# SparseBLAS/spblas-reference

Measured on AMD Instinct MI355X. Metric: csr_spmv_gflops, higher is better.
Workload: dtype f32; 1 GPU; cfg2: fp32 CSR SpMV 10000000x10000000, exactly 10 nnz/row, uniform random unsorted columns, int32 indices, nnz=100000000; rows=10000000, cols=10000000, nnz=100000000, index_type=int32, parallelism=single GPU, operand=matrix_opt(csr_view) + multiply_inspect, alg=auto, plan_alg=3, plan_bytes=1204259164

## Files before the change

spblas-reference_amd/csrc/spmv_sliced.hip:

```cpp
#include <algorithm>
#include <atomic>
#include <type_traits>
#include <vector>

#include "common.hpp"
#include "plan.hpp"
#include "scan.hpp"

#include <cstdlib>
#include <ctime>

namespace spb {

int spmv_hot_build(spblas_gfx950_handle_t h, spblas_gfx950_plan_s* pl, const void* values, bool auto_mode);
int spmv_hot_exec(spblas_gfx950_handle_t h, spblas_gfx950_plan_s* pl, const void* alpha, const void* x, const void* beta,
                  void* y);
int spmv_hot_rows(spblas_gfx950_handle_t h, spblas_gfx950_plan_s* pl, const void* alpha, const void* x, void* y);
int spmv_hot_update(spblas_gfx950_handle_t h, spblas_gfx950_plan_s* pl, const void* values);
void spmv_hot_free(spblas_gfx950_handle_t h, spblas_gfx950_plan_s* pl);
void spmv_sliced_free(spblas_gfx950_handle_t h, spblas_gfx950_plan_s* pl);

static int env_int(const char* name, int dflt) {
  const char* v = std::getenv(name);
  return v && *v ? std::atoi(v) : dflt;
// ... 1468 lines not shown
      }
    }
  };
  if (g_hi > g_lo) {
    batch_t qa, qb;
    issue(g_lo, qa);
    for (int g = g_lo; g < g_hi; g += 2 * UB) {
      issue(g + UB, qb);
      consume(g, qa);
      issue(g + 2 * UB, qa);
      consume(g + UB, qb);
    }
  }
  if (dbg & 2)
    *dummy = dbg_sum;
  if (ENC8 && item.y == 0 && !(dbg & 3)) {
    const int ne = exc_cnt[wb];
    for (int i = lane; i < ne; i += 64) {
      const unsigned e = exc_idx[(size_t) wb * exc_cap + i];
      unsafeAtomicAdd(acc + exc_row[(size_t) wb * exc_cap + i], P[e]);
    }
  }
  if (partial) {
    T* dst = ritems ? partial : partial + (int64_t) blockIdx.y * pstride + r0;
    for (int i0 = lane; i0 < rh; i0 += 64 * 8) {
      T v[8];
#pragma unroll
      for (int u = 0; u < 8; ++u)
        v[u] = acc[i0 + 64 * u < rh ? i0 + 64 * u : 0];
#pragma unroll
      for (int u = 0; u < 8; ++u)
        if (i0 + 64 * u < rh)
          dst[i0 + 64 * u] = v[u];
    }
    return;
  }
  if (peers) {
    for (int i0 = lane; i0 < rh; i0 += 64 * 8) {
      T v[8];
#pragma unroll
      for (int u = 0; u < 8; ++u)
        v[u] = alpha * acc[i0 + 64 * u < rh ? i0 + 64 * u : 0];
      for (int p = 0; p < n_peers; ++p) {
        T* dst = peers[p] + peer_off + r0;
#pragma unroll
        for (int u = 0; u < 8; ++u)
          if (i0 + 64 * u < rh)
            dst[i0 + 64 * u] = v[u];
      }
    }
    return;
  }
  if (rowmap) {
    for (int i = lane; i < rh; i += 64) {
      const T v = alpha * acc[i];
      const int32_t r = rowmap[r0 + i];
      if (r < 0)
        piece_out[r0 + i] = v;
      else
        y[r] = beta == T(0) ? v : v + beta * y[r];
    }
    return;
  }
  for (int i0 = lane; i0 < rh; i0 += 64 * 8) {
    T v[8];
#pragma unroll
    for (int u = 0; u < 8; ++u) {
      const int i = i0 + 64 * u;
      v[u] = alpha * acc[i < rh ? i : 0];
    }
#pragma unroll
    for (int u = 0; u < 8; ++u) {
      const int i = i0 + 64 * u;
      if (i < rh)
        y[r0 + i] = beta == T(0) ? v[u] : v[u] + beta * y[r0 + i];
    }
  }
}


#ifndef PB_VF_GLDS_AUX
#define PB_VF_GLDS_AUX 2
#endif
template <typename T, int NW, int UB, bool ENC8>
__global__ __launch_bounds__(NW * 64) void pb_reduce_vf_kernel(int64_t m, int Hw, int64_t wb_begin, int64_t wb_end,
                                                               const int32_t* __restrict__ binblk, const T* __restrict__ P,
                                                               const uint16_t* __restrict__ s_row,
                                                               const uint16_t* __restrict__ s_src,
                                                               const T* __restrict__ values, const void* __restrict__ rowptr,
                                                               int o64, T* __restrict__ y, T alpha, T beta, int win_cap,
                                                               const typename pb_hdr<T>::type* __restrict__ s_hdr,
                                                               const unsigned* __restrict__ exc_idx,
                                                               const uint16_t* __restrict__ exc_row,
                                                               const int32_t* __restrict__ exc_cnt, int exc_cap,
                                                               T* const* __restrict__ peers, int n_peers, int64_t peer_off) {
  extern __shared__ __attribute__((aligned(16))) unsigned char smem[];
  const int tid = threadIdx.x, wave = __builtin_amdgcn_readfirstlane(threadIdx.x >> 6), lane = threadIdx.x & 63;
  T* win = reinterpret_cast<T*>(smem);
  T* const acc0 = win + win_cap;
  T* const acc = acc0 + (size_t) wave * (Hw + 64);
  const int64_t stride = gridDim.x;
  int64_t wb = wb_begin + blockIdx.x;
  if (wb >= wb_end)
    return;
  constexpr int PB_GBLK = pb_geom<T>::GBLK;
  constexpr int LPB = pb_geom<T>::BLK / 4;
  constexpr int VE = 16 / (int) sizeof(T);
  typedef typename pb_hdr<T>::type hdr_t;
  struct batch_t {
    T p[UB][4];
    u16x4 s[UB];
    u16x4 r[UB];
    unsigned cw[UB];
    hdr_t hd[UB];
  };
  T* const dummy = acc + Hw + lane;
  auto row_off = [&](int64_t r) -> int64_t {
    return o64 ? (int64_t) static_cast<const int64_t*>(rowptr)[r] : (int64_t) static_cast<const int32_t*>(rowptr)[r];
  };
  auto wave_range = [&](int64_t b, int& lo, int& hi) {
    const int gb0 = binblk[b] / PB_GBLK, ng = binblk[b + 1] / PB_GBLK - gb0;
    lo = gb0 + (int) ((int64_t) ng * wave / NW);
    hi = gb0 + (int) ((int64_t) ng * (wave + 1) / NW);
  };
  auto issue = [&](int g, int last, batch_t& q) {
#pragma unroll
    for (int u = 0; u < UB; ++u) {
      const int gg = (g + u) < last ? (g + u) : last;
      const unsigned offR = ((unsigned) gg * PB_GRP + 4u * (unsigned) lane) * 2u;
      const unsigned offP = offR * (unsigned) (sizeof(T) / 2);
      pack4<T>::load(reinterpret_cast<const T*>(reinterpret_cast<const char*>(P) + offP), q.p[u]);
      q.s[u] = stream_load(reinterpret_cast<const u16x4*>(reinterpret_cast<const char*>(s_src) + offR));
      if (ENC8) {
        q.cw[u] = stream_load(reinterpret_cast<const unsigned*>(reinterpret_cast<const char*>(s_row) + (offR >> 1)));
        q.hd[u] = stream_load(s_hdr + ((unsigned) gg * (unsigned) PB_GBLK + (unsigned) lane / LPB));
      } else {
        q.r[u] = stream_load(reinterpret_cast<const u16x4*>(reinterpret_cast<const char*>(s_row) + offR));
      }
    }
  };
  int shift = 0;
  auto stage_window = [&](int64_t b) {
#ifdef PB_EXP_VF_NOWIN
    return;
#endif
    const int64_t r0 = b * Hw, r1 = (r0 + Hw) < m ? (r0 + Hw) : m;
    const int64_t p0 = row_off(r0), p1 = row_off(r1);
    const bool vec_ok = (reinterpret_cast<uintptr_t>(values) & 15) == 0;
    const int64_t p_lo = vec_ok ? (p0 & ~(int64_t) (VE - 1)) : p0;
    shift = (int) (p0 - p_lo);
    const int wn = (int) (p1 - p_lo);
    if (vec_ok) {
      typedef T vec_t __attribute__((ext_vector_type(VE)));
      const int nv = wn / VE;
      const vec_t* src = reinterpret_cast<const vec_t*>(values + p_lo);
      const int nchunk = (nv + 63) >> 6;
      for (int c = wave; c < nchunk; c += NW) {
        const int i = c * 64 + lane;
        if (i < nv)
          __builtin_amdgcn_global_load_lds((const __attribute__((address_space(1))) void*) (src + i),
                                           (__attribute__((address_space(3))) void*) (reinterpret_cast<vec_t*>(win) + c * 64),
                                           16, 0, PB_VF_GLDS_AUX);
      }
      for (int i = nv * VE + tid; i < wn; i += NW * 64)
        win[i] = stream_load(values + p_lo + i);
    } else {
      for (int i = tid; i < wn; i += NW * 64)
        win[i] = stream_load(values + p_lo + i);
    }
  };
  auto consume = [&](int g, int g_hi, const batch_t& q) {
    const T* wv = win + shift;
#pragma unroll
    for (int u = 0; u < UB; ++u) {
      if (g + u >= g_hi)
        break;
#ifdef PB_EXP_VF_NOACC
      {
        T t = q.p[u][0] + q.p[u][1] + q.p[u][2] + q.p[u][3] + T(q.s[u][0] ^ q.s[u][1] ^ q.s[u][2] ^ q.s[u][3]);
        if (ENC8)
          t += T(q.cw[u] ^ (unsigned) q.hd[u]);
        else
          t += T(q.r[u][0]);
        *dummy += t;
        continue;
      }
#endif
      T v[4], pr[4];
      T* slot[4];
      bool flagged[4], atomic[4];
#pragma unroll
      for (int j = 0; j < 4; ++j)
        pr[j] = wv[q.s[u][j]];
      if (ENC8) {
        unsigned row[4];
        bool skip[4];
        pb_decode_rows<LPB>(q.cw[u], pb_hdr<T>::base(q.hd[u]), lane, (unsigned) Hw, row, skip);
        const unsigned fl = pb_hdr<T>::flags(q.hd[u]) >> (4 * (lane & (LPB - 1)));
#pragma unroll
        for (int j = 0; j < 4; ++j) {
          atomic[j] = ((fl >> j) & 1u) != 0 && !skip[j];
          flagged[j] = atomic[j] || skip[j];
          slot[j] = acc + row[j];
          v[j] = *slot[j];
        }
      } else {
#pragma unroll
        for (int j = 0; j < 4; ++j) {
          unsigned r = q.r[u][j];
          asm("" : "+v"(r));
          flagged[j] = atomic[j] = r > 0x7FFFu;
          slot[j] = acc + (r & 0x7FFFu);
          v[j] = *slot[j];
        }
      }
#pragma unroll
      for (int j = 0; j < 4; ++j) {
        pr[j] *= q.p[u][j];
        T* w = flagged[j] ? dummy : slot[j];
        *w = v[j] + pr[j];
      }
      if (__builtin_amdgcn_ballot_w64(atomic[0] | atomic[1] | atomic[2] | atomic[3]) != 0) {
#pragma unroll
        for (int j = 0; j < 4; ++j)
          if (atomic[j])
            unsafeAtomicAdd(slot[j], pr[j]);
      }
    }
  };
  auto end_of_bin = [&]() {
    if (ENC8 && wave == 0) {
      const T* wv = win + shift;
      const int ne = exc_cnt[wb];
      for (int i = lane; i < ne; i += 64) {
        const unsigned e = exc_idx[(size_t) wb * exc_cap + i];
        unsafeAtomicAdd(acc + exc_row[(size_t) wb * exc_cap + i], P[e] * wv[s_src[e]]);
      }
    }
    __builtin_amdgcn_s_waitcnt(0xc07f);
    __builtin_amdgcn_s_barrier();
    const int64_t r0 = wb * Hw;
    const int rh = (int) (((r0 + Hw) < m ? (r0 + Hw) : m) - r0);
    for (int i0 = tid; i0 < rh; i0 += NW * 64 * 4) {
      T sum[4];
#pragma unroll
      for (int u = 0; u < 4; ++u) {
        const int i = (i0 + u * NW * 64) < rh ? (i0 + u * NW * 64) : 0;
        T t = acc0[i];
#pragma unroll
        for (int w = 1; w < NW; ++w)
          t += acc0[(size_t) w * (Hw + 64) + i];
        sum[u] = alpha * t;
      }
#pragma unroll
      for (int u = 0; u < 4; ++u) {
        const int i = i0 + u * NW * 64;
        if (i < rh) {
          if (peers) {
            for (int p = 0; p < n_peers; ++p)
              peers[p][peer_off + r0 + i] = sum[u];
          } else {
            y[r0 + i] = beta == T(0) ? sum[u] : sum[u] + beta * y[r0 + i];
          }
#pragma unroll
          for (int w = 0; w < NW; ++w)
            acc0[(size_t) w * (Hw + 64) + i] = T(0);
        }
      }
    }
    wb += stride;
    if (wb < wb_end) {
      stage_window(wb);
      __builtin_amdgcn_s_waitcnt(0);
      __builtin_amdgcn_s_barrier();
    }
  };
  batch_t qa, qb;
  int g_lo, g_hi;
  wave_range(wb, g_lo, g_hi);
  issue(g_lo, g_hi > g_lo ? g_hi - 1 : g_lo, qa);
  for (int i = tid; i < NW * (Hw + 64); i += NW * 64)
    acc0[i] = T(0);
  stage_window(wb);
  __builtin_amdgcn_s_waitcnt(0);
  __builtin_amdgcn_s_barrier();
  for (;;) {
    const int64_t nb = wb + stride;
    int n_lo = g_hi > g_lo ? g_hi - 1 : g_lo, n_hi = n_lo;
    if (nb < wb_end)
      wave_range(nb, n_lo, n_hi);
    const int last = g_hi > g_lo ? g_hi - 1 : g_lo, n_last = n_hi > n_lo ? n_hi - 1 : n_lo;
    int g = g_lo;
    do {
      issue(g + UB, last, qb);
      consume(g, g_hi, qa);
      const bool more = g + 2 * UB < g_hi;
      issue(more ? g + 2 * UB : n_lo, more ? last : n_last, qa);
      consume(g + UB, g_hi, qb);
      g += 2 * UB;
    } while (g < g_hi);
    end_of_bin();
    if (wb >= wb_end)
      break;
    g_lo = n_lo;
    g_hi = n_hi;
  }
}

template <typename T>
static const void* pb_reduce_vf_fn(int nw, int ub, bool enc8) {
#define SPB_VF(NW_, UB_, E_) reinterpret_cast<const void*>(pb_reduce_vf_kernel<T, NW_, UB_, E_>)
  if (enc8) {
    if (nw == 8)
      return ub == 4 ? SPB_VF(8, 4, true) : SPB_VF(8, 2, true);
    return ub == 4 ? SPB_VF(4, 4, true) : SPB_VF(4, 2, true);
  }
  if (nw == 8)
    return ub == 2 ? SPB_VF(8, 2, false) : SPB_VF(8, 4, false);
  return ub == 2 ? SPB_VF(4, 2, false) : SPB_VF(4, 4, false);
#undef SPB_VF
}
template <typename O>
__global__ __launch_bounds__(256) void pb_bin_span_kernel(int64_t m, int H, int64_t NB, const O* __restrict__ rowptr,
                                                          unsigned long long* __restrict__ out,
                                                          const int32_t* __restrict__ binrow = nullptr) {
  const int64_t b = (int64_t) blockIdx.x * 256 + threadIdx.x;
  unsigned long long span = 0;
  if (b < NB) {
    int64_t r0, r1;
    pb_bin_rows(binrow, b, H, m, &r0, &r1);
    if (r0 < m)
      span = (unsigned long long) (rowptr[r1] - rowptr[r0]);
  }
  for (int o = 32; o > 0; o >>= 1) {
    const unsigned long long u = __shfl_xor(span, o, 64);
    span = u > span ? u : span;
  }
  if ((threadIdx.x & 63) == 0 && span > 0)
    atomicMax(out, span);
}

template <typename T>
__global__ __launch_bounds__(256) void pb_combine_kernel(int64_t r_lo, int64_t r_hi, int K,
                                                         const T* __restrict__ partial, int64_t pstride,
                                                         T* __restrict__ y, T alpha, T beta,
                                                         T* const* __restrict__ peers, int n_peers,
                                                         int64_t peer_off, const int32_t* __restrict__ rowmap,
                                                         T* __restrict__ piece_out) {
  int64_t i = r_lo + (int64_t) blockIdx.x * 256 + threadIdx.x;
  if (i >= r_hi)
    return;
  T s = partial[i];
  for (int k = 1; k < K; ++k)
    s += partial[(int64_t) k * pstride + i];
  if (rowmap) {
    const int32_t r = rowmap[i];
    if (r < 0) {
      piece_out[i] = alpha * s;
      return;
    }
    i = r;
  }
  if (peers) {
    for (int p = 0; p < n_peers; ++p)
      peers[p][peer_off + i] = alpha * s;
    return;
  }
  y[i] = beta == T(0) ? alpha * s : alpha * s + beta * y[i];
}

static constexpr int PB_PUB_ROWS = 2048;
template <typename T>
__global__ __launch_bounds__(256) void pb_combine_publish_kernel(int64_t r_lo, int64_t r_hi, int K,
                                                                 const T* __restrict__ partial, int64_t pstride, T alpha,
                                                                 T* const* __restrict__ peers, int n_peers, int64_t peer_off,
                                                                 long long* const* __restrict__ flag_peers, int slot0,
                                                                 int chunks, long long rows_per_chunk, long long step,
                                                                 int* __restrict__ done, long long delay_ticks) {
#pragma unroll
  for (int u = 0; u < PB_PUB_ROWS / 256; ++u) {
    const int64_t i = r_lo + (int64_t) blockIdx.x * PB_PUB_ROWS + u * 256 + threadIdx.x;
    if (i < r_hi) {
      T s = partial[i];
      for (int k = 1; k < K; ++k)
        s += partial[(int64_t) k * pstride + i];
      for (int p = 0; p < n_peers; ++p)
        __hip_atomic_store(peers[p] + peer_off + i, alpha * s, __ATOMIC_RELAXED, __HIP_MEMORY_SCOPE_SYSTEM);
    }
  }
  __builtin_amdgcn_s_waitcnt(0x0f70);
  __syncthreads();
  if (threadIdx.x == 0) {
    const long long first = (long long) blockIdx.x * PB_PUB_ROWS;
    long long c = first / rows_per_chunk;
// ... 821 lines not shown
    uint16_t* er = pl->s_exc_row;
    int32_t *ec = pl->s_exc_cnt, *fail = pl->s_exc_cnt ? pl->s_exc_cnt + NB : nullptr;
    const int32_t *cnt_ = cnt, *aoff_ = aoff, *prel_ = prel, *binblk_ = binblk, *eoff_ = eoff;
    int32_t* bs = static_cast<int32_t*>(pl->s_blksrc);
    const int32_t* bo = bin_order_dev;
    uint16_t* ssrc = pl->s_src;
    const uint16_t* wp = (e8 && q16) ? wpart : nullptr;
    void* args[] = {&mm, &rowptr, &ci, &vp, &W_, &H_, &S_, &NB_, &cnt_, &aoff_, &prel_, &binblk_, &sv, &sc, &sr, &pm, &bd,
                    &hub, &cap_, &rt_, &binrow, &code, &hdr, &ei, &er, &ec, &ecap, &fail, &eoff_, &bs, &bo, &ssrc, &wp};
    return hipLaunchKernel(fn, dim3((unsigned) NB), dim3(PB_STAGE_THREADS), args, (size_t) PB_STAGE_LDS - 64, s);
  };
  if (staged) {
    SPB_HIP(launch_staged(enc8 != 0));
  } else {
    SPB_HIP(hipFuncSetAttribute(reinterpret_cast<const void*>(pb_scatter_kernel<T, O>),
                                hipFuncAttributeMaxDynamicSharedMemorySize, 16384 * 8));
    hipLaunchKernelGGL((pb_scatter_kernel<T, O>), dim3((unsigned) NB), dim3(256), (size_t) S * 8, s, m, rowptr,
                       pl->colind, static_cast<const T*>(values_p), W, H, S, NB, aoff, prel, binblk,
                       static_cast<T*>(pl->s_values), reinterpret_cast<uint16_t*>(pl->s_colind), pl->s_lrow,
                       reinterpret_cast<int32_t*>(pl->s_perm), static_cast<int32_t*>(pl->s_blkdst), pl->hub_len, binrow,
                       static_cast<const int32_t*>(eoff), static_cast<int32_t*>(pl->s_blksrc));
  }
  tr.mark("scatter");
  SPB_HIP(hipFuncSetAttribute(reinterpret_cast<const void*>(pb_flag_dups_kernel),
                              hipFuncAttributeMaxDynamicSharedMemorySize, PB_LDS_BYTES + 16 * 1024));
  SPB_HIP(hipFuncSetAttribute(reinterpret_cast<const void*>(pb_flag_dups8_kernel<T>),
                              hipFuncAttributeMaxDynamicSharedMemorySize, PB_LDS_BYTES + 16 * 1024));
  auto launch_flags = [&]() {
    if (pl->enc8)
      hipLaunchKernelGGL((pb_flag_dups8_kernel<T>), dim3((unsigned) cdiv(NB, PB_FWAVES)), dim3(PB_FTHREADS),
                         (size_t) PB_FWAVES * (size_t) ((H + 64 + 63) & ~63), s, H, (int64_t) NB, binblk, pl->s_code,
                         static_cast<hdr_t*>(pl->s_hdr));
    else
      hipLaunchKernelGGL(pb_flag_dups_kernel, dim3((unsigned) cdiv(NB, PB_FWAVES)), dim3(PB_FTHREADS),
                         (size_t) PB_FWAVES * (size_t) ((H + 63) & ~63), s, H, (int64_t) NB, binblk, pl->s_lrow, PB_GBLK);
  };
  launch_flags();
  SPB_HIP(hipGetLastError());
  int32_t enc_fail = 0;
  if (pl->enc8) {
    if ((rc = readback_add(h, &enc_fail, pl->s_exc_cnt + NB, 4)) || (rc = readback_flush(h)))
      return rc;
  } else {
    SPB_HIP(hipStreamSynchronize(s));
  }
  if (pl->enc8 && (enc_fail || env_int("SPBLAS_GFX950_PB_ENC8_FAIL", 0))) {
    pl->device_bytes -= (size_t) p_pad + hdr_bytes + (size_t) NB * PB_EXC_CAP * 6;
    pl->device_bytes += (size_t) p_pad * 2;
    dev_free(pl->s_code, s);
    dev_free(pl->s_hdr, s);
    dev_free(pl->s_exc_idx, s);
    dev_free(pl->s_exc_row, s);
    dev_free(pl->s_exc_cnt, s);
    pl->s_code = nullptr;
    pl->s_hdr = nullptr;
    pl->s_exc_idx = nullptr;
    pl->s_exc_row = nullptr;
    pl->s_exc_cnt = nullptr;
    pl->enc8 = 0;
    if ((rc = dev_alloc((void**) &pl->s_lrow, (size_t) (p_pad + PB_GRP) * 2, s)))
      return rc;
    SPB_HIP(hipMemsetD16Async(reinterpret_cast<hipDeviceptr_t>(pl->s_lrow), (unsigned short) H, (size_t) (p_pad + PB_GRP), s));
    SPB_HIP(launch_staged(false));
    launch_flags();
    SPB_HIP(hipGetLastError());
    SPB_HIP(hipStreamSynchronize(s));
    tr.mark("fallback to 16-bit rows");
  }
  tr.mark("flags");
  if (tr.on)
    std::fprintf(stderr, "[inspect] arrays: s_val %p s_col %p blkdst %p blksrc %p P %p rows %p hdr %p  (a_pad %lld, p_pad %lld)\n",
                 pl->s_values, pl->s_colind, pl->s_blkdst, pl->s_blksrc, pl->s_products,
                 pl->enc8 ? (void*) pl->s_code : (void*) pl->s_lrow, pl->s_hdr, (long long) a_pad, (long long) p_pad);
  SPB_HIP(hipFuncSetAttribute(reinterpret_cast<const void*>(pb_expand_kernel<T, false>),
                              hipFuncAttributeMaxDynamicSharedMemorySize, xlds > PB_LDS_BYTES ? xlds : PB_LDS_BYTES));
  SPB_HIP(hipFuncSetAttribute(reinterpret_cast<const void*>(pb_expand_kernel<T, true>),
                              hipFuncAttributeMaxDynamicSharedMemorySize, xlds > PB_LDS_BYTES ? xlds : PB_LDS_BYTES));
  if (vfree) {
    SPB_HIP(hipFuncSetAttribute(reinterpret_cast<const void*>(pb_expand_kernel<T, false, true>),
                                hipFuncAttributeMaxDynamicSharedMemorySize, xlds > PB_LDS_BYTES ? xlds : PB_LDS_BYTES));
    SPB_HIP(hipFuncSetAttribute(reinterpret_cast<const void*>(pb_expand_kernel<T, true, true>),
                                hipFuncAttributeMaxDynamicSharedMemorySize, xlds > PB_LDS_BYTES ? xlds : PB_LDS_BYTES));
    for (int ub : {2, 4})
      SPB_HIP(hipFuncSetAttribute(pb_reduce_vf_fn<T>(pl->vf_waves, ub, pl->enc8 != 0), hipFuncAttributeMaxDynamicSharedMemorySize,
                                  VF_LDS));
    return SPBLAS_GFX950_STATUS_SUCCESS;
  }
  for (int ub : {1, 2, 4, 8})
    SPB_HIP(hipFuncSetAttribute(pb_reduce_fn<T>(pl->rwaves, ub, pl->enc8 != 0), hipFuncAttributeMaxDynamicSharedMemorySize,
                                160 * 1024));
  return SPBLAS_GFX950_STATUS_SUCCESS;
}

int spmv_sliced_build(spblas_gfx950_handle_t h, spblas_gfx950_plan_s* pl, const void* values, bool auto_mode) {
  {
    const int hot = env_int("SPBLAS_GFX950_PB_HOT", -1);
    const double avg = pl->m > 0 ? (double) pl->nnz / (double) pl->m : 0.0;
    const bool skewed = (double) pl->max_row_len > 16.0 * avg + 64.0 || pl->empty_rows * 4 > pl->m;
    const int depth = env_int("SPBLAS_GFX950_PB_HOT_DEPTH", 1);
    if (pl->is_child >= 0 && pl->is_child < depth && hot != 0 && h->bin_row_align <= 1 && pl->nnz > 0 &&
        pl->nnz <= INT32_MAX - 8 && pl->m >= 2 &&
        (hot == 1 || (skewed && pl->nnz >= (4 << 20) && env_int("SPBLAS_GFX950_PB_VARBINS", -1) != 0))) {
      const int rc_h = spmv_hot_build(h, pl, values, auto_mode);
      if (rc_h == SPBLAS_GFX950_STATUS_ALLOC_FAILED) {
        spmv_hot_free(h, pl);
        (void) hipGetLastError();
      } else if (rc_h != SPBLAS_GFX950_STATUS_NOT_SUPPORTED) {
        return rc_h;
      }
    }
  }
  const bool f32 = pl->value_type == SPBLAS_GFX950_F32, o32 = pl->offset_type == SPBLAS_GFX950_I32;
  if (f32)
    return o32 ? sliced_build_typed<float, int32_t>(h, pl, values, auto_mode)
               : sliced_build_typed<float, int64_t>(h, pl, values, auto_mode);
  return o32 ? sliced_build_typed<double, int32_t>(h, pl, values, auto_mode)
             : sliced_build_typed<double, int64_t>(h, pl, values, auto_mode);
}

template <typename T>
static int sliced_update_typed(spblas_gfx950_handle_t h, spblas_gfx950_plan_s* pl, const void* values) {
  pl->values_ptr = values;
  const int64_t a_pad = pl->a_entries;
  if (pl->s_placed == 0 || a_pad == 0 || pl->vfree)
    return SPBLAS_GFX950_STATUS_SUCCESS;
  if (pl->s_eoff && pl->n_rblk > 0 && pl->n_slices > 0 && env_int("SPBLAS_GFX950_PB_UPDATE_BINS", 1)) {
    const int cap = (int) ((PB_STAGE_LDS - 1024 - (((size_t) pl->n_slices * 8 + 15) & ~(size_t) 15)) / sizeof(T)) & ~3;
    const bool o32 = pl->offset_type == SPBLAS_GFX950_I32;
    const void* rp = pl->s_nzrow ? pl->s_rowptr_c : pl->rowptr;
    const int64_t rows = pl->s_nzrow ? pl->s_m : pl->m;
    const int32_t* binrow = static_cast<const int32_t*>(pl->s_binrow);
    const void* fn = o32 ? (const void*) pb_refresh_bins_kernel<T, int32_t> : (const void*) pb_refresh_bins_kernel<T, int64_t>;
    static std::atomic<bool> attr_set[64][2] = {};
    const int dev = h->device >= 0 && h->device < 64 ? h->device : 0;
    if (!attr_set[dev][o32 ? 0 : 1].load(std::memory_order_acquire) || h->device >= 64) {
      SPB_HIP(hipFuncSetAttribute(fn, hipFuncAttributeMaxDynamicSharedMemorySize, PB_STAGE_LDS - 1024));
      attr_set[dev][o32 ? 0 : 1].store(true, std::memory_order_release);
    }
    if (o32)
      hipLaunchKernelGGL((pb_refresh_bins_kernel<T, int32_t>), dim3((unsigned) pl->n_rblk), dim3(1024), (size_t) PB_STAGE_LDS - 1024,
                         h->stream, pl->n_slices, pl->n_rblk, pl->rows_per_blk, rows, binrow, static_cast<const int32_t*>(rp),
                         static_cast<const int2*>(pl->s_eoff), reinterpret_cast<const int32_t*>(pl->s_perm),
                         static_cast<const T*>(values), static_cast<T*>(pl->s_values), cap);
    else
      hipLaunchKernelGGL((pb_refresh_bins_kernel<T, int64_t>), dim3((unsigned) pl->n_rblk), dim3(1024), (size_t) PB_STAGE_LDS - 1024,
                         h->stream, pl->n_slices, pl->n_rblk, pl->rows_per_blk, rows, binrow, static_cast<const int64_t*>(rp),
                         static_cast<const int2*>(pl->s_eoff), reinterpret_cast<const int32_t*>(pl->s_perm),
                         static_cast<const T*>(values), static_cast<T*>(pl->s_values), cap);
    SPB_HIP(hipGetLastError());
    return SPBLAS_GFX950_STATUS_SUCCESS;
  }
  hipLaunchKernelGGL((pb_update_values_kernel<T>), dim3((unsigned) cdiv(a_pad, 256)), dim3(256), 0, h->stream, a_pad,
                     reinterpret_cast<const int32_t*>(pl->s_perm), static_cast<const T*>(values),
                     static_cast<T*>(pl->s_values));
  SPB_HIP(hipGetLastError());
  return SPBLAS_GFX950_STATUS_SUCCESS;
}

int spmv_sliced_update(spblas_gfx950_handle_t h, spblas_gfx950_plan_s* pl, const void* values) {
  const bool have_src = pl->rest_plan ? pl->hot_src != nullptr : (pl->vfree || pl->s_perm != nullptr || pl->s_placed == 0);
  if (!have_src && !pl->is_child) {
    if (stream_capturing(h->stream))
      return SPBLAS_GFX950_STATUS_NOT_SUPPORTED;
    if (pl->used && pl->last_stream != h->stream)
      SPB_HIP(hipStreamSynchronize(pl->last_stream));
    const int nt = pl->nt_products, refresh = pl->refresh_each_call;
    spmv_sliced_free(h, pl);
    pl->device_bytes = pl->base_device_bytes;
// ... 161 lines not shown
  int K = pick_ksplit(wb_end - wb_begin, pl->n_rblk > 0 ? pl->p_blocks / pb_geom<T>::GBLK / pl->n_rblk : 0);
  if (h->max_ksplit > 0 && K > h->max_ksplit)
    K = (int) h->max_ksplit;
  if (pl->vfree) {
    if (!pl->values_ptr)
      return SPBLAS_GFX950_STATUS_INVALID_VALUE;
    K = 1;
  }
  int64_t r_lo = wb_begin * pl->rows_per_blk;
  int64_t r_hi = wb_end * pl->rows_per_blk < pl->s_m ? wb_end * pl->rows_per_blk : pl->s_m;
  int64_t o_lo = r_lo, o_hi = r_hi;
  if (pl->s_binrow) {
    if (wb_begin == 0 && wb_end == pl->n_rblk) {
      r_lo = o_lo = 0;
      r_hi = pl->s_m;
      o_hi = pl->m;
    } else {
      const int rc_b = ensure_host_binrow(h, pl);
      if (rc_b)
        return rc_b;
      r_lo = o_lo = pl->h_binrow[wb_begin];
      r_hi = o_hi = pl->h_binrow[wb_end];
      if (pl->h_binrow_orig) {
        o_lo = wb_begin == 0 ? 0 : pl->h_binrow_orig[wb_begin];
        o_hi = pl->h_binrow_orig[wb_end];
      }
    }
  }
  const int32_t* rowmap = static_cast<const int32_t*>(pl->s_nzrow);
  if (peers_p && rowmap)
    return SPBLAS_GFX950_STATUS_NOT_SUPPORTED;
  if (pl->n_split > 0 && !(wb_begin == 0 && wb_end == pl->n_rblk))
    return SPBLAS_GFX950_STATUS_NOT_SUPPORTED;
  T* piece_out = static_cast<T*>(pl->s_piece_out);
  const bool use_items = pl->s_ritems && !peers_p && wb_begin == 0 && wb_end == pl->n_rblk;
  if (!use_items && K > 1 && pl->s_partial_k < K) {
    if (stream_capturing(s))
      return SPBLAS_GFX950_STATUS_NOT_SUPPORTED;
    dev_free(pl->s_partial, s);
    pl->s_partial = nullptr;
    int rc = dev_alloc(&pl->s_partial, (size_t) K * pl->s_m * sizeof(T), s);
    if (rc)
      return rc;
    pl->s_partial_k = K;
  }
  auto wait_hook = [&]() -> int {
    auto& bw = h->bcast_wait;
    if (!peers_p || !bw.flags)
      return SPBLAS_GFX950_STATUS_SUCCESS;
    const int rc_w = launch_step_wait(h, bw.flags, bw.n_peers, bw.step, bw.timeout_ms, bw.status_dev);
    bw.flags = nullptr;
    return rc_w;
  };
  if (pl->vfree) {
    const int32_t* binblk = static_cast<const int32_t*>(pl->s_binblk);
    const T* Pp = static_cast<const T*>(pl->s_products);
    const uint16_t* rowp = pl->enc8 ? reinterpret_cast<const uint16_t*>(pl->s_code) : pl->s_lrow;
    const uint16_t* srcp = pl->s_src;
    const T* vals = static_cast<const T*>(pl->values_ptr);
    const void* rp = pl->rowptr;
    int o64 = pl->offset_type == SPBLAS_GFX950_I32 ? 0 : 1;
    typedef typename pb_hdr<T>::type hdr_t;
    const hdr_t* hdr = static_cast<const hdr_t*>(pl->s_hdr);
    const unsigned* exc_idx = pl->s_exc_idx;
    const uint16_t* exc_row = pl->s_exc_row;
    const int32_t* exc_cnt = pl->s_exc_cnt;
    int exc_cap = pl->exc_cap, Hw = pl->rows_per_blk, cap = pl->vf_win_cap;
    int64_t mm = pl->m;
    T* yp = static_cast<T*>(y);
    T a = alpha, b = beta;
    int UBv = env_int("SPBLAS_GFX950_PB_RBATCH", pl->enc8 ? 2 : 4);
    if (UBv != 2)
      UBv = 4;
    T* const* peers = reinterpret_cast<T* const*>(peers_p);
    void* args[] = {&mm, &Hw, &wb_begin, &wb_end, &binblk, &Pp, &rowp, &srcp, &vals, &rp, &o64, &yp, &a, &b, &cap, &hdr,
                    &exc_idx, &exc_row, &exc_cnt, &exc_cap, &peers, &n_peers, &peer_off};
    const size_t lds = ((size_t) cap + (size_t) pl->vf_waves * (Hw + 64)) * sizeof(T);
    int64_t grid = env_int("SPBLAS_GFX950_PB_VF_GRID", h->num_cus > 0 ? h->num_cus : 256);
    if (grid < 1 || grid > wb_end - wb_begin)
      grid = wb_end - wb_begin;
    const int rc_w = wait_hook();
    if (rc_w)
      return rc_w;
    SPB_HIP(hipLaunchKernel(pb_reduce_vf_fn<T>(pl->vf_waves, UBv, pl->enc8 != 0), dim3((unsigned) grid),
                            dim3(pl->vf_waves * 64), args, lds, s));
  } else {
    const int32_t* binblk = static_cast<const int32_t*>(pl->s_binblk);
    const T* Pp = static_cast<const T*>(pl->s_products);
    const uint16_t* rowp = pl->enc8 ? reinterpret_cast<const uint16_t*>(pl->s_code) : pl->s_lrow;
    typedef typename pb_hdr<T>::type hdr_t;
    const hdr_t* hdr = static_cast<const hdr_t*>(pl->s_hdr);
    const unsigned* exc_idx = pl->s_exc_idx;
    const uint16_t* exc_row = pl->s_exc_row;
    const int32_t* exc_cnt = pl->s_exc_cnt;
    int exc_cap = pl->exc_cap;
    const bool e8 = pl->enc8 != 0;
    T* yp = static_cast<T*>(y);
    T* part = K > 1 ? static_cast<T*>(pl->s_partial) : nullptr;
    int64_t mm = pl->s_m, pstride = pl->s_m;
    int Hw = pl->rows_per_blk, Kk = K;
    T a = alpha, b = beta;
    T* const* peers = reinterpret_cast<T* const*>(peers_p);
    const int4* ritems = nullptr;
    int dbg = env_int("SPBLAS_GFX950_PB_DBG", 0);
    const int32_t* binrow = static_cast<const int32_t*>(pl->s_binrow);
    void* args[] = {&mm, &Hw, &wb_begin, &wb_end, &binblk, &Pp, &rowp, &yp, &a, &b, &Kk, &part, &pstride,
                    &peers, &n_peers, &peer_off, &ritems, &dbg, &binrow, &rowmap, &piece_out, &hdr, &exc_idx,
                    &exc_row, &exc_cnt, &exc_cap};
    const size_t lds = (size_t) RW * (pl->rows_per_blk + 64) * sizeof(T);
    if (use_items) {
      ritems = static_cast<const int4*>(pl->s_ritems);
      part = static_cast<T*>(pl->s_rpartial);
      pstride = 0;
      SPB_HIP(hipLaunchKernel(pb_reduce_fn<T>(RW, UB, e8), dim3((unsigned) pl->n_ritems), dim3(RW * 64), args, lds, s));
      if (pl->n_rsplit > 0)
        hipLaunchKernelGGL((pb_combine_items_kernel<T>),
                           dim3((unsigned) pl->n_rsplit, (unsigned) cdiv((int64_t) RW * pl->rows_per_blk, 256)), dim3(256),
                           0, s, static_cast<const int4*>(pl->s_rsplit), (int64_t) RW * pl->rows_per_blk, pl->s_m,
                           static_cast<const T*>(pl->s_rpartial), static_cast<T*>(y), alpha, beta, pl->rows_per_blk,
                           binrow, pl->n_rblk, rowmap, piece_out);
    } else {
      if (!(K > 1 && r_hi > r_lo)) {
        const int rc_w = wait_hook();
        if (rc_w)
          return rc_w;
      }
      SPB_HIP(hipLaunchKernel(pb_reduce_fn<T>(RW, UB, e8), dim3((unsigned) groups, (unsigned) K), dim3(RW * 64), args, lds, s));
      if (K > 1 && r_hi > r_lo) {
        const int rc_w = wait_hook();
        if (rc_w)
          return rc_w;
      }
      if (K > 1 && r_hi > r_lo && h->chunk_pub.flag_peers && peers_p && !rowmap) {
        const auto cp = h->chunk_pub;
        h->chunk_pub.flag_peers = nullptr;
        hipLaunchKernelGGL((pb_combine_publish_kernel<T>), dim3((unsigned) cdiv(r_hi - r_lo, PB_PUB_ROWS)), dim3(256), 0, s, r_lo, r_hi,
                           K, static_cast<const T*>(pl->s_partial), pl->s_m, alpha, reinterpret_cast<T* const*>(peers_p),
                           n_peers, peer_off, reinterpret_cast<long long* const*>(cp.flag_peers), cp.slot0, cp.chunks,
                           cp.rows_per_chunk, cp.step, h->chunk_done, cp.delay_ticks);
      } else if (K > 1 && r_hi > r_lo)
        hipLaunchKernelGGL((pb_combine_kernel<T>), dim3((unsigned) cdiv(r_hi - r_lo, 256)), dim3(256), 0, s, r_lo, r_hi, K,
                           static_cast<const T*>(pl->s_partial), pl->s_m, static_cast<T*>(y), alpha, beta,
                           reinterpret_cast<T* const*>(peers_p), n_peers, peer_off, rowmap, piece_out);
    }
  }
  if (pl->n_split > 0)
    hipLaunchKernelGGL((pb_split_finish_kernel<T>), dim3((unsigned) cdiv(pl->n_split, 4)), dim3(256), 0, s, pl->n_split,
                       static_cast<const int4*>(pl->s_split_rows), static_cast<const T*>(piece_out), static_cast<T*>(y), beta);
  if (rowmap && pl->n_zero > 0 && o_hi > o_lo)
    hipLaunchKernelGGL((pb_empty_rows_kernel<T>), dim3((unsigned) cdiv(pl->n_zero, 256)), dim3(256), 0, s, pl->n_zero,
                       static_cast<const int32_t*>(pl->s_zrow), static_cast<T*>(y), beta, o_lo, o_hi);
  if (pl->hub_len > 0 && pl->n_hub > 0) {
    if (!pl->values_ptr || !pl->last_x)
      return SPBLAS_GFX950_STATUS_INVALID_VALUE;
    if (!pl->s_hub_part)
      return SPBLAS_GFX950_STATUS_INVALID_VALUE;
    const dim3 grid((unsigned) pl->n_hub, (unsigned) pl->hub_parts);
    T* part = static_cast<T*>(pl->s_hub_part);
    const int32_t* hub_rows = static_cast<const int32_t*>(pl->s_hub_rows);
    const void* hub_rowptr = rowmap ? pl->s_rowptr_c : pl->rowptr;
    if (pl->offset_type == SPBLAS_GFX950_I32)
      hipLaunchKernelGGL((pb_hub_rows_kernel<T, int32_t>), grid, dim3(256), 0, s, pl->n_hub, hub_rows,
                         static_cast<const int32_t*>(hub_rowptr), pl->colind, static_cast<const T*>(pl->values_ptr),
                         static_cast<const T*>(pl->last_x), part, r_lo, r_hi);
    else
      hipLaunchKernelGGL((pb_hub_rows_kernel<T, int64_t>), grid, dim3(256), 0, s, pl->n_hub, hub_rows,
                         static_cast<const int64_t*>(hub_rowptr), pl->colind, static_cast<const T*>(pl->values_ptr),
// ... 161 lines not shown
```

Measured before the change: 645.0 GFLOP/s.

## Deepen reduce-kernel prefetch pipeline and overlap next window staging with bin writeback

Adds a compile-time pipeline depth D to the value-free reduce kernel and selects D=4 by default, so up to D-1 batches of product, source and row-code loads stay in flight across bins instead of ping-ponging two buffers. The vectorised global-to-LDS copy of the next bin's value window is now issued right after the barrier, before the accumulator reduction and y writeback, so it overlaps that tail; the scalar remainder is staged after. The LDS copy goes through inline asm with an explicit nt hint, and peer stores are cast to the global address space. The extra in-flight batches raise register pressure and may lower occupancy, and the hand-written m0 asm is more fragile.

```diff
diff --git a/spblas-reference_amd/csrc/spmv_sliced.hip b/spblas-reference_amd/csrc/spmv_sliced.hip
--- a/spblas-reference_amd/csrc/spmv_sliced.hip
+++ b/spblas-reference_amd/csrc/spmv_sliced.hip
@@ -1574,7 +1574,15 @@
 #ifndef PB_VF_GLDS_AUX
 #define PB_VF_GLDS_AUX 2
 #endif
-template <typename T, int NW, int UB, bool ENC8>
+static __device__ __forceinline__ void pb_glds16_unseen(const void* src, __attribute__((address_space(3))) void* dst) {
+  static_assert(PB_VF_GLDS_AUX == 2, "the statement below spells the non-temporal hint out");
+  unsigned keep;
+  asm volatile("s_mov_b32 %0, m0\n\ts_mov_b32 m0, %2\n\ts_nop 0\n\tglobal_load_lds_dwordx4 %1, off nt\n\ts_mov_b32 m0, %0"
+               : "=&s"(keep)
+               : "v"(src), "s"((unsigned) (uintptr_t) dst)
+               : "memory");
+}
+template <typename T, int NW, int UB, bool ENC8, int D>
 __global__ __launch_bounds__(NW * 64) void pb_reduce_vf_kernel(int64_t m, int Hw, int64_t wb_begin, int64_t wb_end,
                                                                const int32_t* __restrict__ binblk, const T* __restrict__ P,
                                                                const uint16_t* __restrict__ s_row,
@@ -1632,7 +1640,7 @@
     }
   };
   int shift = 0;
-  auto stage_window = [&](int64_t b) {
+  auto stage_window = [&](int64_t b, int part = 0) {
 #ifdef PB_EXP_VF_NOWIN
     return;
 #endif
@@ -1647,21 +1655,25 @@
       const int nv = wn / VE;
       const vec_t* src = reinterpret_cast<const vec_t*>(values + p_lo);
       const int nchunk = (nv + 63) >> 6;
-      for (int c = wave; c < nchunk; c += NW) {
+      for (int c = wave; c < nchunk && part != 2; c += NW) {
         const int i = c * 64 + lane;
-        if (i < nv)
-          __builtin_amdgcn_global_load_lds((const __attribute__((address_space(1))) void*) (src + i),
-                                           (__attribute__((address_space(3))) void*) (reinterpret_cast<vec_t*>(win) + c * 64),
-                                           16, 0, PB_VF_GLDS_AUX);
-      }
-      for (int i = nv * VE + tid; i < wn; i += NW * 64)
+        if (i < nv) {
+          if (D > 2)
+            pb_glds16_unseen(src + i, (__attribute__((address_space(3))) void*) (reinterpret_cast<vec_t*>(win) + c * 64));
+          else
+            __builtin_amdgcn_global_load_lds((const __attribute__((address_space(1))) void*) (src + i),
+                                             (__attribute__((address_space(3))) void*) (reinterpret_cast<vec_t*>(win) + c * 64),
+                                             16, 0, PB_VF_GLDS_AUX);
+        }
+      }
+      for (int i = nv * VE + tid; i < wn && part != 1; i += NW * 64)
         win[i] = stream_load(values + p_lo + i);
     } else {
-      for (int i = tid; i < wn; i += NW * 64)
+      for (int i = tid; i < wn && part != 1; i += NW * 64)
         win[i] = stream_load(values + p_lo + i);
     }
   };
-  auto consume = [&](int g, int g_hi, const batch_t& q) {
+  auto consume =[&](int g, int g_hi, const batch_t& q) {
     const T* wv = win + shift;
 #pragma unroll
     for (int u = 0; u < UB; ++u) {
@@ -1731,6 +1743,8 @@
     }
     __builtin_amdgcn_s_waitcnt(0xc07f);
     __builtin_amdgcn_s_barrier();
+    if (D > 2 && wb + stride < wb_end)
+      stage_window(wb + stride, 1);
     const int64_t r0 = wb * Hw;
     const int rh = (int) (((r0 + Hw) < m ? (r0 + Hw) : m) - r0);
     for (int i0 = tid; i0 < rh; i0 += NW * 64 * 4) {
@@ -1749,8 +1763,12 @@
         const int i = i0 + u * NW * 64;
         if (i < rh) {
           if (peers) {
-            for (int p = 0; p < n_peers; ++p)
-              peers[p][peer_off + r0 + i] = sum[u];
+            for (int p = 0; p < n_peers; ++p) {
+              if (D > 2)
+                ((__attribute__((address_space(1))) T*) peers[p])[peer_off + r0 + i] = sum[u];
+              else
+                peers[p][peer_off + r0 + i] = sum[u];
+            }
           } else {
             y[r0 + i] = beta == T(0) ? sum[u] : sum[u] + beta * y[r0 + i];
           }
@@ -1761,22 +1779,32 @@
       }
     }
     wb += stride;
-    if (wb < wb_end) {
+    if (D > 2 && wb < wb_end)
+      stage_window(wb, 2);
+    if (D == 2 && wb < wb_end) {
       stage_window(wb);
       __builtin_amdgcn_s_waitcnt(0);
       __builtin_amdgcn_s_barrier();
     }
   };
-  batch_t qa, qb;
+  batch_t q[D];
   int g_lo, g_hi;
   wave_range(wb, g_lo, g_hi);
-  issue(g_lo, g_hi > g_lo ? g_hi - 1 : g_lo, qa);
+#pragma unroll
+  for (int k = 0; k < D - 1; ++k)
+    issue(g_lo + k * UB, g_hi > g_lo ? g_hi - 1 : g_lo, q[k]);
   for (int i = tid; i < NW * (Hw + 64); i += NW * 64)
     acc0[i] = T(0);
   stage_window(wb);
-  __builtin_amdgcn_s_waitcnt(0);
-  __builtin_amdgcn_s_barrier();
+  if (D == 2) {
+    __builtin_amdgcn_s_waitcnt(0);
+    __builtin_amdgcn_s_barrier();
+  }
   for (;;) {
+    if (D > 2) {
+      __builtin_amdgcn_s_waitcnt(0);
+      __builtin_amdgcn_s_barrier();
+    }
     const int64_t nb = wb + stride;
     int n_lo = g_hi > g_lo ? g_hi - 1 : g_lo, n_hi = n_lo;
     if (nb < wb_end)
@@ -1784,12 +1812,14 @@
     const int last = g_hi > g_lo ? g_hi - 1 : g_lo, n_last = n_hi > n_lo ? n_hi - 1 : n_lo;
     int g = g_lo;
     do {
-      issue(g + UB, last, qb);
-      consume(g, g_hi, qa);
-      const bool more = g + 2 * UB < g_hi;
-      issue(more ? g + 2 * UB : n_lo, more ? last : n_last, qa);
-      consume(g + UB, g_hi, qb);
-      g += 2 * UB;
+      const bool more = g + D * UB < g_hi;
+#pragma unroll
+      for (int k = 0; k < D; ++k) {
+        const bool here = k == 0 || more;
+        issue(here ? g + (k + D - 1) * UB : n_lo + (k - 1) * UB, here ? last : n_last, q[(k + D - 1) % D]);
+        consume(g + k * UB, g_hi, q[k]);
+      }
+      g += D * UB;
     } while (g < g_hi);
     end_of_bin();
     if (wb >= wb_end)
@@ -1800,8 +1830,10 @@
 }
 
 template <typename T>
-static const void* pb_reduce_vf_fn(int nw, int ub, bool enc8) {
-#define SPB_VF(NW_, UB_, E_) reinterpret_cast<const void*>(pb_reduce_vf_kernel<T, NW_, UB_, E_>)
+static const void* pb_reduce_vf_fn(int nw, int ub, bool enc8, int depth) {
+#define SPB_VF(NW_, UB_, E_) \
+  (depth == 2 ? reinterpret_cast<const void*>(pb_reduce_vf_kernel<T, NW_, UB_, E_, 2>) \
+              : reinterpret_cast<const void*>(pb_reduce_vf_kernel<T, NW_, UB_, E_, 4>))
   if (enc8) {
     if (nw == 8)
       return ub == 4 ? SPB_VF(8, 4, true) : SPB_VF(8, 2, true);
@@ -2789,8 +2821,9 @@
     SPB_HIP(hipFuncSetAttribute(reinterpret_cast<const void*>(pb_expand_kernel<T, true, true>),
                                 hipFuncAttributeMaxDynamicSharedMemorySize, xlds > PB_LDS_BYTES ? xlds : PB_LDS_BYTES));
     for (int ub : {2, 4})
-      SPB_HIP(hipFuncSetAttribute(pb_reduce_vf_fn<T>(pl->vf_waves, ub, pl->enc8 != 0), hipFuncAttributeMaxDynamicSharedMemorySize,
-                                  VF_LDS));
+      for (int depth : {2, 4})
+        SPB_HIP(hipFuncSetAttribute(pb_reduce_vf_fn<T>(pl->vf_waves, ub, pl->enc8 != 0, depth),
+                                    hipFuncAttributeMaxDynamicSharedMemorySize, VF_LDS));
     return SPBLAS_GFX950_STATUS_SUCCESS;
   }
   for (int ub : {1, 2, 4, 8})
@@ -3118,7 +3151,8 @@
     const int rc_w = wait_hook();
     if (rc_w)
       return rc_w;
-    SPB_HIP(hipLaunchKernel(pb_reduce_vf_fn<T>(pl->vf_waves, UBv, pl->enc8 != 0), dim3((unsigned) grid),
+    const int depth = env_int("SPBLAS_GFX950_PB_VF_DEPTH", 4) == 2 ? 2 : 4;
+    SPB_HIP(hipLaunchKernel(pb_reduce_vf_fn<T>(pl->vf_waves, UBv, pl->enc8 != 0, depth), dim3((unsigned) grid),
                             dim3(pl->vf_waves * 64), args, lds, s));
   } else {
     const int32_t* binblk = static_cast<const int32_t*>(pl->s_binblk);
```

New measurement: 644.5 GFLOP/s. Within noise of the previous version (-0.1%).
